# scjjb/HIPT_ABMIL_ATEC23

Measured on AMD Instinct MI355X. Metric: 4K-regions/sec HIPT extract + ABMIL fwd ms @100k×384; 1/2/4/8 MI355X, higher is better.
Workload: dtype bf16; 1 GPU; per step: HIPT_4K.forward on R resident [3,4096,4096] fp32 regions (R x 256 patches ViT-256 -> ViT-4K over each 16x16 [CLS] grid, BASELINE configs[2]) + CLAM_SB gated-attention pooling over one 100000x384 bag (configs[3], the bag resident in the compute dtype); random-init weights of the reference architectures; streams=3, input=fp32 normalised, bag_dtype=bf16-resident, chunk_patches=2048, parallelism=slide-sharded x1, one all-gather

## Files before the change

### hipt_abmil_atec23_amd/_native.py

```python
from __future__ import annotations

import ctypes as C
import os
import subprocess
import threading

HERE = os.path.dirname(os.path.abspath(__file__))
LIB_PATH = os.environ.get("HIPT_AMD_LIB") or os.path.join(HERE, "libhipt_abmil.so")
CSRC = os.path.join(HERE, "csrc")

HIPT_F32, HIPT_BF16 = 0, 1
EPI_GELU, EPI_RESID, EPI_OUT_F32, EPI_RELU = 1, 2, 4, 16
ABI_VERSION = 6
PACK_QKV, PACK_PROJ, PACK_MLP, PACK_QKV_ATT, PACK_CLS_ABSORB = 0, 1, 2, 3, 4
CLS_ABSORB_TAIL = 0x4B564142

c_f32p = C.c_void_p


class BlockWeights(C.Structure):
    _fields_ = [(n, C.c_void_p) for n in (
        "ln1_w", "ln1_b", "qkv_w", "qkv_b", "proj_w", "proj_b",
        "ln2_w", "ln2_b", "fc1_w", "fc1_b", "fc2_w", "fc2_b", "qkv_pk", "proj_pk", "mlp_pk")] + [
        ("mlp_pk_fmt", C.c_int32), ("cls_absorb", C.c_int32), ("qkv_att_pk", C.c_void_p)]
# ... 69 lines not shown
    "hipt_abi_version": (_i, []),
    "hipt_last_error": (C.c_char_p, []),
    "hipt_profile_enable": (_i, [_i]),
    "hipt_profile_categories": (_i, []),
    "hipt_profile_category_name": (C.c_char_p, [_i]),
    "hipt_profile_read": (_i, [_p, _p]),
    "hipt_layernorm": (_i, [_p, _i64, _p, _p, _p, _i, _i64, _i, _i, _f, _p]),
    "hipt_linear": (_i, [_p, _i64, _p, _i64, _p, _p, _p, _i64, _i, _i, _i, _i, _i, _p]),
    "hipt_attention": (_i, [_p, _p, _p, _i, _i, _i, _i, _f, _i, _p]),
    "hipt_vit_workspace_bytes": (_sz, [_VW, _i]),
    "hipt_vit_packed_bytes": (_sz, [_VW, _i]),
    "hipt_vit_mlp_pack_format": (_i, [_VW]),
    "hipt_vit_pack_weights": (_i, [_VW, _i, _i, _p, _p]),
    "hipt_vit256_forward_workspace_bytes": (_sz, [_VW, _IL, _i, _i]),
    "hipt_vit4k_forward_workspace_bytes": (_sz, [_VW, _i]),
    "hipt_vit256_prepare_tokens": (_i, [_VW, _p, _IL, _i, _i, _p, _p, _sz, _p]),
    "hipt_vit4k_prepare_tokens": (_i, [_VW, _p, _i, _p, _p, _sz, _p]),
    "hipt_vit_blocks": (_i, [_VW, _p, _i, _i, _i, _p, _p, _sz, _p]),
    "hipt_vit_head": (_i, [_VW, _p, _i, _i, _p, _p]),
    "hipt_vit_cls_attention": (_i, [_VW, _p, _i, _p, _p, _sz, _p]),
    "hipt_vit_attention_unit": (_i, [_VW, _i, _p, _i, _p, _i, _p, _sz, _p]),
    "hipt_vit_mlp_unit": (_i, [_VW, _i, _p, _p, _i, _p, _p, _sz, _p]),
    "hipt_vit_cls_block_unit": (_i, [_VW, _p, _p, _i, _p, _p, _p, _sz, _p]),
    "hipt_vit_embed_unit": (_i, [_VW, _p, _i, _IL, _i, _i, _p, _p, _p, _sz, _p]),
    "hipt_vit256_forward": (_i, [_VW, _p, _IL, _i, _i, _p, _p, _sz, _p]),
    "hipt_vit4k_forward": (_i, [_VW, _p, _i, _p, _p, _sz, _p]),
    "hipt_image_compute_bytes": (_sz, [_VW, _IL, _i, _i]),
    "hipt_image_to_compute": (_i, [_VW, _p, _i, _IL, _i, _p, _p]),
    "hipt_vit256_range_workspace_bytes": (_sz, [_VW, _i, _i]),
    "hipt_vit256_forward_range": (_i, [_VW, _p, _IL, _i, _i, _i, _p, _p, _sz, _p]),
    "hipt_vit256_range_px_workspace_bytes": (_sz, [_VW, _IL, _i, _i]),
    "hipt_vit256_forward_range_px": (_i, [_VW, _p, _IL, _i, _i, _i, _p, _p, _sz, _p]),
    "hipt_hipt4k_workspace_bytes": (_sz, [_VW, _VW, _i, _i, _i, _i]),
    "hipt_hipt4k_forward": (_i, [_VW, _VW, _p, _i, _i, _i, _i, _p, _p, _p, _sz, _p]),
    "hipt_hipt4k_u8_workspace_bytes": (_sz, [_VW, _VW, _i, _i, _i, _i]),
    "hipt_hipt4k_forward_u8": (_i, [_VW, _VW, _p, _i, _i, _i, _i, _i, _p, _p, _p, _sz, _p]),
    "hipt_u8_normalize": (_i, [_p, _i, C.c_int64, C.c_int64, _p, _i, _p]),
    "hipt_clam_workspace_bytes": (_sz, [_CW, _i]),
    "hipt_clam_stream_packed_bytes": (_sz, [_CW]),
    "hipt_clam_stream_pack": (_i, [_CW, _p, _p]),
    "hipt_clam_ticket_offset": (_sz, [_CW, _i]),
    "hipt_clam_sb_forward": (_i, [_CW, _p, _i, _i, _p, _p, _p, _p, _p, _p, _sz, _p]),
    "hipt_clam_bags_supported": (_i, [_CW]),
    "hipt_clam_bags_workspace_bytes": (_sz, [_CW, _i, _i64]),
    "hipt_clam_sb_forward_bags": (_i, [_CW, _p, _p, _i, _i64, _i, _p, _p, _p, _p, _p, _p, _sz, _p]),
    "hipt_clam_wide_bags_supported": (_i, [_CW]),
# ... 183 lines not shown
```

### hipt_abmil_atec23_amd/csrc/capi.hip

```cpp
#include <stdarg.h>
#include <stdio.h>
#include <stdlib.h>
#include <string.h>

#include "common.h"
#include "kernels.h"
#include "workspace.h"

static thread_local char g_err[512] = "";

void hipt_set_error(const char* fmt, ...) {
    va_list ap;
    va_start(ap, fmt);
    vsnprintf(g_err, sizeof(g_err), fmt, ap);
    va_end(ap);
}

namespace {

inline int esz(int dtype) { return dtype == HIPT_F32 ? 4 : 2; }
inline hipStream_t S(void* s) { return (hipStream_t)s; }

enum { PC_EMBED, PC_LN, PC_QKV, PC_ATTN, PC_PROJ, PC_FC1, PC_FC2, PC_MLP, PC_ABMIL, PC_COMBINE, PC_OTHER, PC_VIT4K, PC_LASTCLS, PC_QKVATT, PC_CLSROWS, PC_N };
const char* const kProfNames[PC_N] = {"embed_gemm", "layernorm", "qkv_gemm", "attention", "proj_gemm",
// ... 90 lines not shown
    const hipt_block_weights& b = w->blocks[blk];
    const int D = w->dim;
    SeqGemmParams q;
    memset(&q, 0, sizeof(q));
    q.M = M; q.K = D; q.ln_eps = w->ln_eps;
    q.A = x; q.lda = D; q.ln_w = b.ln1_w; q.ln_b = b.ln1_b; q.W = b.qkv_w; q.wpk = b.qkv_pk; q.N = 3 * D; q.bias = b.qkv_b;
    q.out = s.qkv; q.ldc = 3 * D; q.out_ntok = w->ntok;
    q.counter = s.queues->qkv;
    return q;
}
inline void qkv_from_xn(SeqGemmParams& q, const void* xn) { q.A = xn, q.ln_w = q.ln_b = nullptr; }

MlpParams mlp_params(const hipt_vit_weights* w, int blk, int M, float* x, const BlockScratch& s) {
    const hipt_block_weights& b = w->blocks[blk];
    MlpParams m;
    memset(&m, 0, sizeof(m));
    m.x = x; m.y1 = s.xn; m.bproj = b.proj_b; m.ln_w = b.ln2_w; m.ln_b = b.ln2_b; m.ln_eps = w->ln_eps;
    m.w1 = b.fc1_w; m.b1 = b.fc1_b; m.w2 = b.fc2_w; m.b2 = b.fc2_b; m.wpk = b.mlp_pk; m.wpk_fmt = b.mlp_pk_fmt; m.M = M; m.D = w->dim; m.hidden = w->hidden;
    m.counter = s.queues->mlp;
    return m;
}
inline void mlp_emit_xn(MlpParams& m, const hipt_block_weights& next, void* xn_out) { m.ln_next_w = next.ln1_w, m.ln_next_b = next.ln1_b, m.xn_out = xn_out; }

int rows_linear(GemmParams p, int dtype, int flags, hipStream_t st, int a_row_step = 0, void* gather = nullptr) {
    p.asc = 1;
    if (a_row_step > 0) {
        if (!hipt_generic_only() && hipt_gemm_arows_supported(p.M, p.K, dtype, ALOAD_PLAIN, 0)) {
            p.a_row_step = a_row_step;
        } else {
            int rc = hipt_gather_cls_bf16_launch(p.A, gather, p.M, a_row_step, p.K, st, 1);
            if (rc) return rc;
            p.A = gather;
        }
    }
    return linear(p, dtype, flags, st);
}

static bool small_call(const hipt_vit_weights* w, int nseq) { return (int64_t)nseq * w->ntok <= 1088; }

static bool blocks_chain(const hipt_vit_weights* w, int nseq, int b0, int b1) {
    const int D = w->dim, dt = w->dtype;
    bool chain = hipt_seqgemm_supported(dt, D) && hipt_mlp_supported(dt, D, w->hidden) && !small_call(w, nseq) && !hipt_generic_only() &&
                 hipt_mlp16_supported(dt, D, w->hidden) && hipt_seqgemm_pipe_supported(dt, D, 3 * D, false, 0);
    for (int i = b0; i < b1 && chain; ++i) chain = w->blocks[i].qkv_pk && w->blocks[i].proj_pk && w->blocks[i].mlp_pk && (w->blocks[i].mlp_pk_fmt == 2 || w->blocks[i].mlp_pk_fmt == 3);
    return chain;
}

static bool can_prune_last(const hipt_vit_weights* w) {
    return w->dtype == HIPT_BF16 && w->dim == 384 && w->dim / w->heads == 64 && w->ntok <= 320 && hipt_seqgemm_supported(w->dtype, w->dim) &&
           hipt_mlp_supported(w->dtype, w->dim, w->hidden) && !hipt_env_on("HIPT_NO_PRUNE");
}

enum {
    RT_EMIT_LAST = 1,
    RT_CLS_ONLY = 2,
    RT_PX_EMBED = 4,
    RT_FORCE_SMALL = 8,
};
struct VitRoute {
    int b0, b1;
    bool emit_last;
    bool small, force_small;
    bool seq;
    bool chain;
    bool img;
    bool hm;
    bool prune;
    bool pre;
    bool fuse_ok, fold_ok, absorb_ok;
    bool have_xn = false;
    bool x_img = false;
};

VitRoute vit_route(const hipt_vit_weights* w, int nseq, int b0, int b1, bool want_probs, int accept) {
    const int D = w->dim, dt = w->dtype;
    const int64_t M = (int64_t)nseq * w->ntok;
    VitRoute r;
    r.force_small = (accept & RT_FORCE_SMALL) != 0;
    r.small = small_call(w, nseq) || r.force_small;
    r.prune = (accept & RT_CLS_ONLY) && can_prune_last(w) && !small_call(w, nseq);
    r.b0 = b0;
    r.b1 = r.prune ? w->depth - 1 : b1;
    r.emit_last = r.prune || (accept & RT_EMIT_LAST);
    r.seq = hipt_seqgemm_supported(dt, D) && hipt_mlp_supported(dt, D, w->hidden) && !r.small;
    r.chain = !r.force_small && blocks_chain(w, nseq, r.b0, r.b1);
    r.img = r.chain && r.prune && !want_probs && M % 16 == 0 && !hipt_env_on("HIPT_NO_IMG") && hipt_attention64_supported(dt, D / w->heads, w->ntok, false);
    r.hm = r.img && M * 3 * D * 2 < ((int64_t)1 << 32) - 65536;
    r.pre = r.img && (accept & RT_PX_EMBED) && r.b0 < r.b1 && !hipt_env_on("HIPT_NO_EMBED_LN");
    r.fuse_ok = hipt_qkv_attn_supported(dt, D, w->heads, w->ntok) && !hipt_env_on("HIPT_NO_FUSED_ATTN");
    r.fold_ok = r.chain && !hipt_env_on("HIPT_NO_PROJ_FOLD");
    r.absorb_ok = hipt_cls_pool_supported(dt, D, w->heads, w->ntok) && !hipt_env_on("HIPT_NO_CLS_ABSORB");
    return r;
}

struct BlockRoute {
    bool fuse;
    bool fold;
    bool absorb;
};
BlockRoute block_route(const VitRoute& r, const hipt_block_weights& b, bool last_probs) {
    BlockRoute k;
    k.fuse = r.have_xn && r.x_img && b.qkv_att_pk && r.fuse_ok && !last_probs;
    k.fold = r.fold_ok && b.mlp_pk_fmt == 3 && !last_probs;
    k.absorb = k.fuse && b.cls_absorb == HIPT_CLS_ABSORB_TAIL && r.absorb_ok;
    return k;
}

int cls_rows_qkv(const hipt_vit_weights* w, const hipt_block_weights& b, int nseq, int N, const BlockScratch& s, int a_row_step, hipStream_t st) {
    const int D = w->dim;
    return rows_linear(gemm_params(a_row_step > 0 ? s.att : s.cls_xn, D, b.qkv_w, D, b.qkv_b, s.cls_qkv, N, nseq, N, D), w->dtype, 0, st, a_row_step, s.cls_xn);
}

int run_blocks(const hipt_vit_weights* w, float* x, int nseq, float* probs, const BlockScratch& s, VitRoute& r, hipStream_t st) {
    const int D = w->dim, M = nseq * w->ntok, dt = w->dtype, dh = D / w->heads;
// ... 44 lines not shown
        }
        const bool ln_al = (((uintptr_t)b.ln1_w | (uintptr_t)b.ln1_b | (uintptr_t)b.ln2_w | (uintptr_t)b.ln2_b) & 15) == 0;
        const bool ln_in_gemm = r.small && ln_al && !hipt_generic_only() && hipt_gemm_ln_supported(M, D, ALOAD_PLAIN, 0, r.force_small);
        auto lin = [&](int cat, GemmParams g, int flags) -> int {
            g.rpt = w->ntok;
            g.small_any = r.force_small ? 1 : 0;
            if (flags & HIPT_EPI_RESID) g.resid = x;
            PROF(cat, linear(g, dt, flags, st));
            return HIPT_OK;
        };
        auto ln_lin = [&](int cat, const float* lw, const float* lb, GemmParams g, int flags) -> int {
            if (ln_in_gemm) {
                g.ln_w = lw; g.ln_b = lb; g.ln_eps = w->ln_eps;
            } else {
                PROF(PC_LN, hipt_layernorm_launch(x, D, lw, lb, s.xn, dt, D, M, D, w->ln_eps, st));
                g.A = s.xn;
            }
            return lin(cat, g, flags);
        };
        const int H = w->hidden;
        if ((rc = ln_lin(PC_QKV, b.ln1_w, b.ln1_b, gemm_params(x, D, b.qkv_w, D, b.qkv_b, s.qkv, 3 * D, M, 3 * D, D), 0))) return rc;
        PROF(PC_ATTN, hipt_attention_launch(s.qkv, s.att, last_probs ? probs : nullptr, nseq, w->ntok, w->heads, dh, scale, dt, st));
        if (last_probs) break;
        if ((rc = lin(PC_PROJ, gemm_params(s.att, D, b.proj_w, D, b.proj_b, x, D, M, D, D), HIPT_EPI_RESID | HIPT_EPI_OUT_F32))) return rc;
        if ((rc = ln_lin(PC_FC1, b.ln2_w, b.ln2_b, gemm_params(x, D, b.fc1_w, D, b.fc1_b, s.hid, H, M, H, D), HIPT_EPI_GELU))) return rc;
        if ((rc = lin(PC_FC2, gemm_params(s.hid, H, b.fc2_w, H, b.fc2_b, x, D, M, D, H), HIPT_EPI_RESID | HIPT_EPI_OUT_F32))) return rc;
    }
    return HIPT_OK;
}

static int run_last_block_cls(const hipt_vit_weights* w, float* x, int nseq, const BlockScratch& s, const VitRoute& r, hipStream_t st) {
    const int D = w->dim, M = nseq * w->ntok, dt = w->dtype, last = w->depth - 1;
    const hipt_block_weights& b = w->blocks[last];
    const float scale = attn_scale(w);
    const BlockRoute k = block_route(r, b, false);
    int rc;
    const void* att_rows = s.att;
    if (k.fuse) {
        PROF(PC_LASTCLS, hipt_gather_cls_bf16_launch(s.att, s.cls_xn, nseq, w->ntok, D, st, 1));
        if (k.absorb) {
            const int HD = w->heads * D;
            const char* wu = (const char*)b.qkv_att_pk + hipt_qkv_attn_packed_bytes();
            const char* wo = wu + (size_t)HD * D * 2;
            PROF(PC_LASTCLS, cls_rows_qkv(w, b, nseq, D, s, 0, st));
            PROF(PC_LASTCLS, rows_linear(gemm_params(s.cls_qkv, D, wu, D, nullptr, s.u, HD, nseq, HD, D), dt, HIPT_EPI_OUT_F32, st));
            PROF(PC_LASTCLS, hipt_cls_pool_launch(s.att, (const float*)s.u, s.z, nseq, scale, st));
            PROF(PC_LASTCLS, rows_linear(gemm_params(s.z, HD, wo, HD, b.qkv_b + 2 * D, s.qkv, D, nseq, D, HD), dt, 0, st));
        } else {
            PROF(PC_LASTCLS, cls_rows_qkv(w, b, nseq, 3 * D, s, 0, st));
            PROF(PC_LASTCLS, hipt_qkv_attn_cls_launch(s.att, b.qkv_att_pk, b.qkv_b, s.cls_qkv, s.qkv, nseq, scale, st));
        }
        att_rows = s.qkv;
    } else {
        SeqGemmParams q = qkv_params(w, last, M, x, s);
        if (r.have_xn) {
            PROF(PC_LASTCLS, hipt_gather_cls_bf16_launch(s.att, s.cls_xn, nseq, w->ntok, D, st, r.x_img ? 1 : 0));
            const size_t wq = (size_t)D * D * 2;
            qkv_from_xn(q, s.att);
            q.img = r.x_img ? 1 : 0;
            q.W = (const char*)b.qkv_w + wq; q.wpk = b.qkv_pk ? (const char*)b.qkv_pk + wq : nullptr; q.N = 2 * D; q.bias = b.qkv_b + D;
            q.out = (bf16_t*)s.qkv + D;
            PROF(PC_LASTCLS, hipt_seqgemm_launch(q, false, 0, st));
            q.img = 0;
            q.M = nseq; q.A = s.cls_xn; q.W = b.qkv_w; q.wpk = b.qkv_pk; q.N = D; q.bias = b.qkv_b; q.out = s.qkv; q.ldc = w->ntok * 3 * D;
            q.counter = s.queues->aux;
            PROF(PC_LASTCLS, hipt_seqgemm_launch(q, false, 0, st));
        } else {
            PROF(PC_QKV, hipt_seqgemm_launch(q, true, 0, st));
        }
        PROF(PC_LASTCLS, hipt_attn_cls_launch(s.qkv, s.att, nullptr, nseq, w->ntok, w->heads, D / w->heads, scale, st));
    }
    PROF(PC_OTHER, hipt_gather_cls_launch(x, s.xc, nseq, (int64_t)w->ntok * D, D, st, r.x_img ? 1 : 0));
    PROF(PC_LASTCLS, rows_linear(gemm_params(att_rows, D, b.proj_w, D, b.proj_b, s.xn, D, nseq, D, D), dt, 0, st));
    PROF(PC_LASTCLS, hipt_mlp_launch(mlp_params(w, last, nseq, s.xc, s), st));
    return HIPT_OK;
}

int64_t image_elems(const hipt_image_layout* lay, int nseq_total) {
    const int per = lay->grid_w * lay->grid_h;
    return (int64_t)((nseq_total + per - 1) / per) * lay->batch_stride;
}

enum { IMG_F32 = 0, IMG_U8_CHW = 1, IMG_U8_HWC = 2 };

size_t image_compute_bytes(const hipt_vit_weights* w, const hipt_image_layout* lay, int nseq, int kind) {
    const size_t n = (size_t)image_elems(lay, nseq);
    return w->dtype == HIPT_BF16 ? al256(n * 2) : kind != IMG_F32 ? al256(n * 4) : 0;
}

int embed256(const hipt_vit_weights* w, const void* img, const hipt_image_layout* lay, int seq0, int nseq, float* x,
             hipStream_t st) {
    HIPT_CHECK_ARG(lay->patch_h % 16 == 0 && lay->patch_w % 16 == 0, "vit256: patch %dx%d not a multiple of 16", lay->patch_h,
                   lay->patch_w);
    const int nty = lay->patch_h / 16, ntx = lay->patch_w / 16;
// ... 308 lines not shown
    m.y1 = att_img;
    m.fold = 1;
    m.img = 3;
    if (xn_out_img) mlp_emit_xn(m, w->blocks[block + 1 < w->depth ? block + 1 : block], xn_out_img);
    hipStream_t st = S(stream);
    PROF(PC_MLP, hipt_mlp_launch(m, st));
    return HIPT_OK;
}

int hipt_vit_cls_block_unit(const hipt_vit_weights* w, const void* xn_img, const float* x_img, int nseq, float* xc_out, void* att_out, void* workspace,
                            size_t ws_bytes, void* stream) {
    int rc = check_vit(w);
    if (rc) return rc;
    HIPT_CHECK_ARG(xn_img && x_img && xc_out && nseq > 0, "vit_cls_block_unit: null/empty argument");
    const int D = w->dim;
    const int64_t M = (int64_t)nseq * w->ntok;
    VitRoute r = vit_route(w, nseq, 0, w->depth, false, RT_CLS_ONLY | RT_PX_EMBED);
    if (!hipt_qkv_attn_supported(w->dtype, D, w->heads, w->ntok) || M % 16 != 0 || !r.prune || !r.chain || !r.img) {
        hipt_set_error("vit_cls_block_unit: bf16, D = 384, 6 heads, 257 tokens, nseq * 257 %% 16 == 0 and a forward that prunes its last block "
                       "on activation images only");
        return HIPT_E_UNSUPPORTED;
    }
    r.have_xn = r.x_img = true;
    Carver c(workspace, workspace ? ws_bytes : 0);
    BlockScratch s = carve_vit4k(c, w, nseq, false).s;
    if ((rc = check_workspace(c, "vit_cls_block_unit"))) return rc;
    HIPT_CHECK_ARG(s.fits_cls_xn, "vit_cls_block_unit: hidden %d leaves no room for the [CLS] rows in the block scratch", w->hidden);
    hipStream_t st = S(stream);
    if (block_route(r, w->blocks[w->depth - 1], false).fuse)
        s.att = const_cast<void*>(xn_img);
    else if (hipMemcpyAsync(s.att, xn_img, (size_t)M * D * 2, hipMemcpyDeviceToDevice, st) != hipSuccess)
        return HIPT_E_LAUNCH;
    const void* rows = s.att == xn_img ? s.qkv : s.att;
    if ((rc = run_last_block_cls(w, const_cast<float*>(x_img), nseq, s, r, st))) return rc;
    if (hipMemcpyAsync(xc_out, s.xc, (size_t)nseq * D * 4, hipMemcpyDeviceToDevice, st) != hipSuccess) return HIPT_E_LAUNCH;
    if (att_out && hipMemcpyAsync(att_out, rows, (size_t)nseq * D * 2, hipMemcpyDeviceToDevice, st) != hipSuccess) return HIPT_E_LAUNCH;
    return HIPT_OK;
}

int hipt_vit_embed_unit(const hipt_vit_weights* w, const void* images, int input_kind, const hipt_image_layout* lay, int seq0, int nseq, float* x_out,
                        void* xn_out_img, void* workspace, size_t ws_bytes, void* stream) {
    int rc = check_vit(w);
    if (rc) return rc;
    HIPT_CHECK_ARG(images && lay && x_out && nseq > 0 && seq0 >= 0 && input_kind >= IMG_F32 && input_kind <= IMG_U8_HWC && (!xn_out_img || w->depth > 0),
                   "vit_embed_unit: bad argument");
    if (!embed_fused_ok(w, images, lay, embed_px_slot_bytes(), input_kind) || (xn_out_img && ((int64_t)nseq * w->ntok) % 16 != 0)) {
        hipt_set_error("vit_embed_unit: bf16, D = 384, 256 x 256 patches of 16 x 16-pixel tokens, 16-byte aligned pixel rows (uint8: strides %% 8 == 0, "
                       "batch_stride = 3 * chan_stride), nseq * ntok %% 16 == 0 for the image outputs, and not under HIPT_GENERIC only");
        return HIPT_E_UNSUPPORTED;
    }
    Carver c(workspace, workspace ? ws_bytes : 0);
    void* slot = c.take(embed_px_slot_bytes());
    if ((rc = check_workspace(c, "vit_embed_unit"))) return rc;
    hipStream_t st = S(stream);
    if ((rc = hipt_embed32_pack_launch(w->embed_w, slot, st))) return rc;
    return embed256_px(w, images, input_kind, lay, seq0, nseq, x_out, slot, xn_out_img, st);
}

int hipt_vit_mlp_pack_format(const hipt_vit_weights* w) { return w && hipt_mlp16_supported(w->dtype, w->dim, w->hidden) ? 3 : 0; }
// ... 47 lines not shown
}

static int vit256_range_impl(const hipt_vit_weights* w, const void* img, const hipt_image_layout* lay, int seq0, int nseq, int chunk, float* out,
                             void* workspace, size_t ws_bytes, hipStream_t st, const void* embed_pk = nullptr, int embed_kind = IMG_F32) {
    int rc;
    const int D = w->dim;
    Carver c(workspace, ws_bytes);
    const RangeWs g = carve_range(c, w, nseq, chunk);
    if ((rc = check_workspace(c, "vit256_forward"))) return rc;
    for (int s0 = 0; s0 < nseq; s0 += g.chunk) {
        const int n = nseq - s0 < g.chunk ? nseq - s0 : g.chunk;
        VitRoute r = vit_route(w, n, 0, w->depth, false, RT_CLS_ONLY | (embed_pk ? RT_PX_EMBED : 0));
        if (r.prune && !(r.chain ? g.s.fits_cls_xn : g.s.fits_xc)) {
            hipt_set_error("vit256_forward: %d tokens x hidden %d leave no room in the block scratch for the [CLS] rows of the pruned last block "
                           "(HIPT_NO_PRUNE=1 runs it in full)", w->ntok, w->hidden);
            return HIPT_E_WORKSPACE;
        }
        if (embed_pk)
            rc = embed256_px(w, img, embed_kind, lay, seq0 + s0, n, g.x, embed_pk, r.pre ? g.s.att : nullptr, st);
        else
            rc = embed256(w, img, lay, seq0 + s0, n, g.x, st);
        if (rc) return rc;
        if ((rc = run_blocks(w, g.x, n, nullptr, g.s, r, st))) return rc;
        if (r.prune && (rc = run_last_block_cls(w, g.x, n, g.s, r, st))) return rc;
        PROF(PC_LN, hipt_layernorm_launch(r.prune ? g.s.xc : g.x, r.prune ? D : (int64_t)w->ntok * D, w->norm_w, w->norm_b, out + (size_t)s0 * D,
                                          HIPT_F32, D, n, D, w->ln_eps, st));
    }
    return HIPT_OK;
}

static int image_to_compute(const hipt_vit_weights* w, const void* images, int kind, const hipt_image_layout* lay, int nseq, void* dst,
                            const void** img_out, hipStream_t st) {
    int rc;
    const int64_t n_img = image_elems(lay, nseq);
    if (kind != IMG_F32) {
        const int per = lay->grid_w * lay->grid_h;
        HIPT_CHECK_ARG(nseq % per == 0, "vit256_forward: uint8 input must hold whole regions");
        const int64_t plane = lay->batch_stride / 3;
        PROF(PC_OTHER, hipt_u8_normalize_launch(images, kind == IMG_U8_HWC, nseq / per, plane, dst, w->dtype, st));
        *img_out = dst;
    } else if (w->dtype == HIPT_BF16) {
        PROF(PC_OTHER, hipt_f32_to_bf16_launch((const float*)images, dst, n_img, st));
        *img_out = dst;
    } else {
        *img_out = images;
    }
    return HIPT_OK;
// ... 363 lines not shown
```

### hipt_abmil_atec23_amd/csrc/kernels.h

```cpp
#pragma once
#include <hip/hip_runtime.h>
#include <stdint.h>

#include "../../include/hipt_abmil.h"

enum { ALOAD_PLAIN = 0, ALOAD_IM2COL = 1 };
enum { EPI_ROWMAP = 32 };

struct GemmParams {
    const void* A;
    int64_t lda;
    const void* W;
    int64_t ldw;
    int M, N, K;
    int rpt;
    const float* bias;
    const float* resid;
    void* out;
    int64_t ldc;
    const float* pos;
    int rows_per_seq;
    hipt_image_layout im;
    int im_nty, im_ntx, im_seq0;
    const float *ln_w, *ln_b;
// ... 88 lines not shown
bool hipt_mlp16_supported(int dtype, int D, int hidden);
int hipt_mlp16_launch(const MlpParams& p, hipStream_t st);
size_t hipt_mlp16_packed_bytes(int D, int hidden, bool with_proj);
int hipt_mlp16_pack_launch(const void* w1, const void* w2, int D, int hidden, void* packed, hipStream_t st, const void* wproj = nullptr);

int hipt_layernorm_launch(const float* x, int64_t x_stride, const float* w, const float* b, void* out, int out_dtype,
                          int64_t out_stride, int rows, int D, float eps, hipStream_t st);

int hipt_attention_launch(const void* qkv, void* out, float* probs, int B, int ntok, int heads, int dh, float scale,
                          int dtype, hipStream_t st, int out_img = 0, int qkv_hm = 0);
bool hipt_attention64_supported(int dtype, int dh, int ntok, bool want_probs);
int hipt_attention64_launch(const void* qkv, void* out, int B, int ntok, int heads, float scale, hipStream_t st, int out_img = 0, int qkv_hm = 0);

bool hipt_qkv_attn_supported(int dtype, int D, int heads, int ntok);
size_t hipt_qkv_attn_packed_bytes();
int hipt_qkv_attn_pack_launch(const void* qkv_w, void* packed, hipStream_t st);
int hipt_qkv_attn_launch(const void* xn_img, const void* wpk, const float* qkv_b, const void* qkv_cls, void* out_img, int nseq, float scale, hipStream_t st);
int hipt_qkv_attn_cls_launch(const void* xn_img, const void* wpk, const float* qkv_b, const void* qkv_cls, void* out_rows, int nseq, float scale, hipStream_t st);

bool hipt_cls_pool_supported(int dtype, int D, int heads, int ntok);
size_t hipt_cls_absorb_packed_bytes();
int hipt_cls_absorb_pack_launch(const void* qkv_w, void* packed, hipStream_t st);
int hipt_cls_pool_launch(const void* xn_img, const float* u, void* z, int nseq, float scale, hipStream_t st);

int hipt_attn_cls_launch(const void* qkv, void* out, float* probs, int B, int ntok, int heads, int dh, float scale, hipStream_t st);
int hipt_attn_cls_probs_launch(const void* qkv, float* probs, int B, int ntok, int heads, int dh, float scale, int dtype, hipStream_t st);
int hipt_gather_cls_launch(const float* src, float* dst, int nseq, int64_t seq_stride, int D, hipStream_t st, int img = 0);
int hipt_gather_cls_bf16_launch(const void* src, void* dst, int nseq, int ntok, int D, hipStream_t st, int img = 0);
int hipt_cls_init_launch(float* x, const float* cls, const float* pos, int nseq, int ntok, int D, hipStream_t st);
int hipt_cls_init_img_launch(float* x_img, void* xn_img, const float* cls, const float* pos, const float* ln_w, const float* ln_b, float ln_eps, int nseq,
                             int ntok, int D, hipStream_t st);
int hipt_add_bf16_launch(float* out, const float* src, const void* y, int64_t n, hipStream_t st);
int hipt_u8_normalize_launch(const void* src, int hwc, int64_t nimg, int64_t plane, void* dst, int dst_dtype, hipStream_t st);
int hipt_f32_to_bf16_launch(const float* in, void* out, int64_t n, hipStream_t st);

bool hipt_clam_fused_supported(const hipt_clam_weights* w);
int hipt_clam_fused_launch(const hipt_clam_weights* w, const void* bag, int N, int attention_only, float* A_raw,
                           float* partials, int* n_partials, hipStream_t st);
bool hipt_clam_stream_supported(const hipt_clam_weights* w);
size_t hipt_clam_stream_image_bytes(const hipt_clam_weights* w);
int hipt_clam_stream_pack_launch(const hipt_clam_weights* w, void* out, hipStream_t st);
int hipt_clam_stream_launch(const hipt_clam_weights* w, const void* bag, int N, int attention_only, float* A_raw,
                            float* partials, int* n_partials, unsigned* ticket, float* M, float* logits, float* Y_prob,
                            int64_t* Y_hat, hipStream_t st);
bool hipt_clam_mb_stream_supported(const hipt_clam_weights* w);
size_t hipt_clam_mb_h1_bytes(int N);
// ... 36 lines not shown
```

### include/hipt_abmil.h

```cpp
#ifndef HIPT_ABMIL_H
#define HIPT_ABMIL_H

#include <stddef.h>
#include <stdint.h>

#ifdef __cplusplus
extern "C" {
#endif

#define HIPT_ABI_VERSION 6

enum { HIPT_F32 = 0, HIPT_BF16 = 1 };

enum {
    HIPT_OK = 0,
    HIPT_E_BADARG = -1,
    HIPT_E_WORKSPACE = -2,
    HIPT_E_LAUNCH = -3,
    HIPT_E_UNSUPPORTED = -4
};

int hipt_abi_version(void);
const char* hipt_last_error(void);

// ... 69 lines not shown
size_t hipt_vit256_forward_workspace_bytes(const hipt_vit_weights* w, const hipt_image_layout* lay,
                                           int nseq, int chunk);
size_t hipt_vit4k_forward_workspace_bytes(const hipt_vit_weights* w, int nseq);

int hipt_vit256_prepare_tokens(const hipt_vit_weights* w, const float* images,
                               const hipt_image_layout* lay, int seq0, int nseq, float* x,
                               void* workspace, size_t ws_bytes, void* stream);

int hipt_vit4k_prepare_tokens(const hipt_vit_weights* w, const float* tokens_in, int nseq, float* x,
                              void* workspace, size_t ws_bytes, void* stream);

int hipt_vit_blocks(const hipt_vit_weights* w, float* x, int nseq, int blk_begin, int blk_end,
                    float* probs, void* workspace, size_t ws_bytes, void* stream);

int hipt_vit_attention_unit(const hipt_vit_weights* w, int block, const void* xn_img, int nseq, void* out_img, int fused,
                            void* workspace, size_t ws_bytes, void* stream);

int hipt_vit_mlp_unit(const hipt_vit_weights* w, int block, float* x_img, const void* att_img, int nseq, void* xn_out_img,
                      void* workspace, size_t ws_bytes, void* stream);

int hipt_vit_cls_block_unit(const hipt_vit_weights* w, const void* xn_img, const float* x_img, int nseq, float* xc_out, void* att_out,
                            void* workspace, size_t ws_bytes, void* stream);

int hipt_vit_embed_unit(const hipt_vit_weights* w, const void* images, int input_kind, const hipt_image_layout* lay, int seq0, int nseq,
                        float* x_out, void* xn_out_img, void* workspace, size_t ws_bytes, void* stream);

int hipt_vit_cls_attention(const hipt_vit_weights* w, float* x, int nseq, float* probs_cls,
                           void* workspace, size_t ws_bytes, void* stream);

int hipt_vit_head(const hipt_vit_weights* w, const float* x, int nseq, int cls_only, float* out,
                  void* stream);

int hipt_vit256_forward(const hipt_vit_weights* w, const float* images, const hipt_image_layout* lay,
                        int nseq, int chunk, float* out, void* workspace, size_t ws_bytes, void* stream);

size_t hipt_image_compute_bytes(const hipt_vit_weights* w, const hipt_image_layout* lay, int nseq, int input_kind);
int hipt_image_to_compute(const hipt_vit_weights* w, const void* images, int input_kind, const hipt_image_layout* lay,
                          int nseq, void* dst, void* stream);
size_t hipt_vit256_range_workspace_bytes(const hipt_vit_weights* w, int nseq, int chunk);
int hipt_vit256_forward_range(const hipt_vit_weights* w, const void* images_cd, const hipt_image_layout* lay,
                              int seq0, int nseq, int chunk, float* out, void* workspace, size_t ws_bytes, void* stream);
size_t hipt_vit256_range_px_workspace_bytes(const hipt_vit_weights* w, const hipt_image_layout* lay, int nseq, int chunk);
int hipt_vit256_forward_range_px(const hipt_vit_weights* w, const float* images, const hipt_image_layout* lay, int seq0, int nseq,
                                 int chunk, float* out, void* workspace, size_t ws_bytes, void* stream);

int hipt_vit4k_forward(const hipt_vit_weights* w, const float* tokens_in, int nseq, float* out,
// ... 306 lines not shown
```

Before: 339.5 regions/s.

## Fuse proj, LN2, MLP and final norm into one per-row chain kernel

Adds a row_chain kernel that runs, for 16-row tiles, the attention output projection with residual, LayerNorm2, FC1+GELU, FC2 with residual, and optionally a leading absorbed-value GEMM and the final norm, keeping intermediates in LDS. It is used for the small ViT-4K block path and the last-block CLS rows of ViT-256, replacing several GEMM, gather and layernorm launches. The aim is to cut launch overhead and intermediate memory traffic on the small-M stages. The cost is that each block streams the full weight matrices for only 16 rows, so weight reuse is low and few workgroups are launched for small M.

```diff
diff --git a/hipt_abmil_atec23_amd/_native.py b/hipt_abmil_atec23_amd/_native.py
--- a/hipt_abmil_atec23_amd/_native.py
+++ b/hipt_abmil_atec23_amd/_native.py
@@ -115,6 +115,7 @@
     "hipt_vit_attention_unit": (_i, [_VW, _i, _p, _i, _p, _i, _p, _sz, _p]),
     "hipt_vit_mlp_unit": (_i, [_VW, _i, _p, _p, _i, _p, _p, _sz, _p]),
     "hipt_vit_cls_block_unit": (_i, [_VW, _p, _p, _i, _p, _p, _p, _sz, _p]),
+    "hipt_row_chain_unit": (_i, [_VW, _i, _p, _p, _p, _p, _i64, _i, _i, _p, _i, _p]),
     "hipt_vit_embed_unit": (_i, [_VW, _p, _i, _IL, _i, _i, _p, _p, _p, _sz, _p]),
     "hipt_vit256_forward": (_i, [_VW, _p, _IL, _i, _i, _p, _p, _sz, _p]),
     "hipt_vit4k_forward": (_i, [_VW, _p, _i, _p, _p, _sz, _p]),
diff --git a/hipt_abmil_atec23_amd/csrc/capi.hip b/hipt_abmil_atec23_amd/csrc/capi.hip
--- a/hipt_abmil_atec23_amd/csrc/capi.hip
+++ b/hipt_abmil_atec23_amd/csrc/capi.hip
@@ -136,6 +136,15 @@
 }
 inline void mlp_emit_xn(MlpParams& m, const hipt_block_weights& next, void* xn_out) { m.ln_next_w = next.ln1_w, m.ln_next_b = next.ln1_b, m.xn_out = xn_out; }
 
+RowChainParams chain_params(const hipt_vit_weights* w, const hipt_block_weights& b, int M, const void* a, const float* x, int64_t x_row_step, int x_img, float* out) {
+    RowChainParams c;
+    memset(&c, 0, sizeof(c));
+    c.a = a; c.lda = w->dim; c.x = x; c.x_row_step = x_row_step; c.x_img = x_img; c.out = out; c.M = M;
+    c.proj_w = b.proj_w; c.proj_b = b.proj_b; c.ln_w = b.ln2_w; c.ln_b = b.ln2_b; c.ln_eps = w->ln_eps;
+    c.fc1_w = b.fc1_w; c.fc1_b = b.fc1_b; c.fc2_w = b.fc2_w; c.fc2_b = b.fc2_b;
+    return c;
+}
+
 int rows_linear(GemmParams p, int dtype, int flags, hipStream_t st, int a_row_step = 0, void* gather = nullptr) {
     p.asc = 1;
     if (a_row_step > 0) {
@@ -182,6 +191,7 @@
     bool prune;
     bool pre;
     bool fuse_ok, fold_ok, absorb_ok;
+    bool row_chain;
     bool have_xn = false;
     bool x_img = false;
 };
@@ -204,6 +214,7 @@
     r.fuse_ok = hipt_qkv_attn_supported(dt, D, w->heads, w->ntok) && !hipt_env_on("HIPT_NO_FUSED_ATTN");
     r.fold_ok = r.chain && !hipt_env_on("HIPT_NO_PROJ_FOLD");
     r.absorb_ok = hipt_cls_pool_supported(dt, D, w->heads, w->ntok) && !hipt_env_on("HIPT_NO_CLS_ABSORB");
+    r.row_chain = hipt_row_chain_supported(dt, D, w->hidden) && !hipt_generic_only() && !hipt_env_on("HIPT_NO_ROW_CHAIN");
     return r;
 }
 
@@ -294,6 +305,13 @@
         if ((rc = ln_lin(PC_QKV, b.ln1_w, b.ln1_b, gemm_params(x, D, b.qkv_w, D, b.qkv_b, s.qkv, 3 * D, M, 3 * D, D), 0))) return rc;
         PROF(PC_ATTN, hipt_attention_launch(s.qkv, s.att, last_probs ? probs : nullptr, nseq, w->ntok, w->heads, dh, scale, dt, st));
         if (last_probs) break;
+        if (r.force_small && r.row_chain) {
+            const RowChainParams c = chain_params(w, b, M, s.att, x, 1, 0, x);
+            if (hipt_row_chain_aligned(c)) {
+                PROF(PC_VIT4K, hipt_row_chain_launch(c, D, st));
+                continue;
+            }
+        }
         if ((rc = lin(PC_PROJ, gemm_params(s.att, D, b.proj_w, D, b.proj_b, x, D, M, D, D), HIPT_EPI_RESID | HIPT_EPI_OUT_F32))) return rc;
         if ((rc = ln_lin(PC_FC1, b.ln2_w, b.ln2_b, gemm_params(x, D, b.fc1_w, D, b.fc1_b, s.hid, H, M, H, D), HIPT_EPI_GELU))) return rc;
         if ((rc = lin(PC_FC2, gemm_params(s.hid, H, b.fc2_w, H, b.fc2_b, x, D, M, D, H), HIPT_EPI_RESID | HIPT_EPI_OUT_F32))) return rc;
@@ -301,13 +319,17 @@
     return HIPT_OK;
 }
 
-static int run_last_block_cls(const hipt_vit_weights* w, float* x, int nseq, const BlockScratch& s, const VitRoute& r, hipStream_t st) {
+static int run_last_block_cls(const hipt_vit_weights* w, float* x, int nseq, const BlockScratch& s, const VitRoute& r, hipStream_t st,
+                              float* norm_out = nullptr, bool* normed = nullptr) {
     const int D = w->dim, M = nseq * w->ntok, dt = w->dtype, last = w->depth - 1;
     const hipt_block_weights& b = w->blocks[last];
     const float scale = attn_scale(w);
     const BlockRoute k = block_route(r, b, false);
     int rc;
     const void* att_rows = s.att;
+    RowChainParams c = chain_params(w, b, nseq, nullptr, x, w->ntok, r.x_img ? 1 : 0, norm_out ? norm_out : s.xc);
+    if (norm_out) c.norm_w = w->norm_w, c.norm_b = w->norm_b;
+    bool chain = r.row_chain;
     if (k.fuse) {
         PROF(PC_LASTCLS, hipt_gather_cls_bf16_launch(s.att, s.cls_xn, nseq, w->ntok, D, st, 1));
         if (k.absorb) {
@@ -317,6 +339,12 @@
             PROF(PC_LASTCLS, cls_rows_qkv(w, b, nseq, D, s, 0, st));
             PROF(PC_LASTCLS, rows_linear(gemm_params(s.cls_qkv, D, wu, D, nullptr, s.u, HD, nseq, HD, D), dt, HIPT_EPI_OUT_F32, st));
             PROF(PC_LASTCLS, hipt_cls_pool_launch(s.att, (const float*)s.u, s.z, nseq, scale, st));
+            c.a = s.z; c.lda = HD; c.lead_w = wo; c.lead_ldw = HD; c.lead_b = b.qkv_b + 2 * D; c.dh = D / w->heads;
+            if ((chain = chain && hipt_row_chain_aligned(c))) {
+                PROF(PC_LASTCLS, hipt_row_chain_launch(c, D, st));
+                if (normed) *normed = norm_out != nullptr;
+                return HIPT_OK;
+            }
             PROF(PC_LASTCLS, rows_linear(gemm_params(s.z, HD, wo, HD, b.qkv_b + 2 * D, s.qkv, D, nseq, D, HD), dt, 0, st));
         } else {
             PROF(PC_LASTCLS, cls_rows_qkv(w, b, nseq, 3 * D, s, 0, st));
@@ -342,6 +370,12 @@
         }
         PROF(PC_LASTCLS, hipt_attn_cls_launch(s.qkv, s.att, nullptr, nseq, w->ntok, w->heads, D / w->heads, scale, st));
     }
+    c.a = att_rows; c.lda = D; c.lead_w = nullptr; c.lead_b = nullptr;
+    if (chain && hipt_row_chain_aligned(c)) {
+        PROF(PC_LASTCLS, hipt_row_chain_launch(c, D, st));
+        if (normed) *normed = norm_out != nullptr;
+        return HIPT_OK;
+    }
     PROF(PC_OTHER, hipt_gather_cls_launch(x, s.xc, nseq, (int64_t)w->ntok * D, D, st, r.x_img ? 1 : 0));
     PROF(PC_LASTCLS, rows_linear(gemm_params(att_rows, D, b.proj_w, D, b.proj_b, s.xn, D, nseq, D, D), dt, 0, st));
     PROF(PC_LASTCLS, hipt_mlp_launch(mlp_params(w, last, nseq, s.xc, s), st));
@@ -696,6 +730,7 @@
         return HIPT_E_UNSUPPORTED;
     }
     r.have_xn = r.x_img = true;
+    r.row_chain = false;
     Carver c(workspace, workspace ? ws_bytes : 0);
     BlockScratch s = carve_vit4k(c, w, nseq, false).s;
     if ((rc = check_workspace(c, "vit_cls_block_unit"))) return rc;
@@ -709,6 +744,24 @@
     if ((rc = run_last_block_cls(w, const_cast<float*>(x_img), nseq, s, r, st))) return rc;
     if (hipMemcpyAsync(xc_out, s.xc, (size_t)nseq * D * 4, hipMemcpyDeviceToDevice, st) != hipSuccess) return HIPT_E_LAUNCH;
     if (att_out && hipMemcpyAsync(att_out, rows, (size_t)nseq * D * 2, hipMemcpyDeviceToDevice, st) != hipSuccess) return HIPT_E_LAUNCH;
+    return HIPT_OK;
+}
+
+int hipt_row_chain_unit(const hipt_vit_weights* w, int block, const void* a, const void* lead_w, const float* lead_b, const float* x, int64_t x_row_step,
+                        int x_img, int final_norm, float* out, int M, void* stream) {
+    int rc = check_vit(w);
+    if (rc) return rc;
+    HIPT_CHECK_ARG(block >= 0 && block < w->depth && a && x && out && M > 0, "row_chain_unit: bad argument");
+    if (!hipt_row_chain_supported(w->dtype, w->dim, w->hidden)) {
+        hipt_set_error("row_chain_unit: bf16, D in {192, 384}, hidden = 4 D only (dtype %d, D = %d, hidden = %d)", w->dtype, w->dim, w->hidden);
+        return HIPT_E_UNSUPPORTED;
+    }
+    const int D = w->dim;
+    RowChainParams c = chain_params(w, w->blocks[block], M, a, x, x_row_step, x_img, out);
+    if (lead_w) c.lda = c.lead_ldw = (int64_t)w->heads * D, c.lead_w = lead_w, c.lead_b = lead_b, c.dh = D / w->heads;
+    if (final_norm) c.norm_w = w->norm_w, c.norm_b = w->norm_b;
+    hipStream_t st = S(stream);
+    PROF(D >= 384 ? PC_LASTCLS : PC_VIT4K, hipt_row_chain_launch(c, D, st));
     return HIPT_OK;
 }
 
@@ -802,7 +855,9 @@
             rc = embed256(w, img, lay, seq0 + s0, n, g.x, st);
         if (rc) return rc;
         if ((rc = run_blocks(w, g.x, n, nullptr, g.s, r, st))) return rc;
-        if (r.prune && (rc = run_last_block_cls(w, g.x, n, g.s, r, st))) return rc;
+        bool normed = false;
+        if (r.prune && (rc = run_last_block_cls(w, g.x, n, g.s, r, st, out + (size_t)s0 * D, &normed))) return rc;
+        if (normed) continue;
         PROF(PC_LN, hipt_layernorm_launch(r.prune ? g.s.xc : g.x, r.prune ? D : (int64_t)w->ntok * D, w->norm_w, w->norm_b, out + (size_t)s0 * D,
                                           HIPT_F32, D, n, D, w->ln_eps, st));
     }
diff --git a/hipt_abmil_atec23_amd/csrc/kernels.h b/hipt_abmil_atec23_amd/csrc/kernels.h
--- a/hipt_abmil_atec23_amd/csrc/kernels.h
+++ b/hipt_abmil_atec23_amd/csrc/kernels.h
@@ -134,6 +134,32 @@
 size_t hipt_cls_absorb_packed_bytes();
 int hipt_cls_absorb_pack_launch(const void* qkv_w, void* packed, hipStream_t st);
 int hipt_cls_pool_launch(const void* xn_img, const float* u, void* z, int nseq, float scale, hipStream_t st);
+
+struct RowChainParams {
+    const void*   a;
+    int64_t lda;
+    const void*   lead_w;
+    int64_t lead_ldw;
+    const float* lead_b;
+    int dh;
+    const float* x;
+    int64_t x_row_step;
+    int x_img;
+    const void*   proj_w;
+    const float* proj_b;
+    const float *ln_w, *ln_b;
+    float ln_eps;
+    const void*   fc1_w;
+    const float* fc1_b;
+    const void*   fc2_w;
+    const float* fc2_b;
+    const float *norm_w, *norm_b;
+    float* out;
+    int M;
+};
+bool hipt_row_chain_supported(int dtype, int D, int hidden);
+bool hipt_row_chain_aligned(const RowChainParams& p);
+int hipt_row_chain_launch(const RowChainParams& p, int D, hipStream_t st);
 
 int hipt_attn_cls_launch(const void* qkv, void* out, float* probs, int B, int ntok, int heads, int dh, float scale, hipStream_t st);
 int hipt_attn_cls_probs_launch(const void* qkv, float* probs, int B, int ntok, int heads, int dh, float scale, int dtype, hipStream_t st);
diff --git a/hipt_abmil_atec23_amd/csrc/row_chain.hip b/hipt_abmil_atec23_amd/csrc/row_chain.hip
--- /dev/null
+++ b/hipt_abmil_atec23_amd/csrc/row_chain.hip
@@ -0,0 +1,262 @@
+#include "common.h"
+#include "kernels.h"
+#include "launch.h"
+#include "mlp_common.h"
+
+namespace {
+
+constexpr int RC_NT = 3;
+
+template <int D> struct RcCfg {
+    static constexpr int H = 4 * D, WAVES = D / (16 * RC_NT), THREADS = 64 * WAVES;
+    static constexpr int APITCH = D * 2 + 16, HPITCH = H * 2 + 16;
+    static constexpr int OFF_H = 16 * APITCH, OFF_ST = OFF_H + 16 * HPITCH, LDS = OFF_ST + 2 * WAVES * 16 * 4;
+    static_assert(D % (16 * RC_NT) == 0 && LDS <= 64 * 1024, "static LDS");
+};
+
+template <int NK, bool AG>
+__device__ __forceinline__ void rc_mm(f32x4 (&acc)[RC_NT], const bf16_t* const (&wp)[RC_NT], const char* const (&ap)[RC_NT]) {
+    constexpr int KU = (NK % 12 == 0 && !AG) ? 6 : 3;
+    static_assert(NK % (2 * KU) == 0, "two register sets in turn");
+    constexpr int NA = AG ? RC_NT : 1;
+    u32x4 w0[KU][RC_NT], w1[KU][RC_NT], a0[KU][NA], a1[KU][NA];
+    auto load = [&](u32x4(&w)[KU][RC_NT], u32x4(&a)[KU][NA], int k0) {
+#pragma unroll
+        for (int d = 0; d < KU; ++d) {
+#pragma unroll
+            for (int t = 0; t < RC_NT; ++t) w[d][t] = *(const u32x4*)(wp[t] + (k0 + d) * 32);
+            if constexpr (AG) {
+#pragma unroll
+                for (int t = 0; t < RC_NT; ++t) a[d][t] = *(const u32x4*)(ap[t] + (k0 + d) * 64);
+            }
+        }
+    };
+    auto mma = [&](const u32x4(&w)[KU][RC_NT], const u32x4(&a)[KU][NA], int k0) {
+#pragma unroll
+        for (int d = 0; d < KU; ++d) {
+            if constexpr (AG) {
+#pragma unroll
+                for (int t = 0; t < RC_NT; ++t) Tr<bf16_t>::mma16(acc[t], w[d][t], a[d][t]);
+            } else {
+                const u32x4 al = *(const u32x4*)(ap[0] + (k0 + d) * 64);
+#pragma unroll
+                for (int t = 0; t < RC_NT; ++t) Tr<bf16_t>::mma16(acc[t], w[d][t], al);
+            }
+        }
+    };
+    load(w0, a0, 0);
+    for (int k0 = 0; k0 < NK; k0 += 2 * KU) {
+        load(w1, a1, k0 + KU);
+        mma(w0, a0, k0);
+        if (k0 + 2 * KU < NK) load(w0, a0, k0 + 2 * KU);
+        mma(w1, a1, k0 + KU);
+    }
+}
+
+template <int D, bool ERF>
+__global__ __launch_bounds__(RcCfg<D>::THREADS) void row_chain_kernel(const RowChainParams p) {
+    using C = RcCfg<D>;
+    constexpr int H = C::H, WAVES = C::WAVES;
+    __shared__ __attribute__((aligned(16))) char smem[C::LDS];
+    const int tid = threadIdx.x, lane = tid & 63, li = lane & 15, g = lane >> 4;
+    const int w = __builtin_amdgcn_readfirstlane(tid >> 6);
+    const int row0 = blockIdx.x * 16;
+    const int row = row0 + li < p.M ? row0 + li : p.M - 1;
+    char* const abuf = smem;
+    char* const hbuf = smem + C::OFF_H;
+    float* const st = (float*)(smem + C::OFF_ST);
+    const int nw = 16 * RC_NT * w;
+
+    f32x4 xr[RC_NT];
+    {
+        const int64_t R = (int64_t)row * p.x_row_step;
+#pragma unroll
+        for (int t = 0; t < RC_NT; ++t) {
+            const int n = nw + 16 * t + 4 * g;
+            if (p.x_img) {
+                const int m = n >> 3;
+                xr[t] = *(const f32x4*)(p.x + (R >> 4) * (16 * D) + (m >> 2) * 512 + ((n >> 2) & 1) * 256 + (16 * (m & 3) + (int)(R & 15)) * 4);
+            } else {
+                xr[t] = *(const f32x4*)(p.x + R * D + n);
+            }
+        }
+    }
+
+    if (p.lead_w) {
+        f32x4 acc[RC_NT];
+        const bf16_t* wp[RC_NT];
+        const char* ap[RC_NT];
+#pragma unroll
+        for (int t = 0; t < RC_NT; ++t) {
+            const int n0 = nw + 16 * t, k0 = (n0 / p.dh) * D;
+            acc[t] = f32x4{0.f, 0.f, 0.f, 0.f};
+            wp[t] = (const bf16_t*)p.lead_w + (int64_t)(n0 + li) * p.lead_ldw + k0 + 8 * g;
+            ap[t] = (const char*)((const bf16_t*)p.a + (int64_t)row * p.lda + k0 + 8 * g);
+        }
+        rc_mm<D / 32, true>(acc, wp, ap);
+#pragma unroll
+        for (int t = 0; t < RC_NT; ++t) {
+            const int n = nw + 16 * t + 4 * g;
+            const f32x4 v = acc[t] + *(const f32x4*)(p.lead_b + n);
+            u32x2 o;
+            o[0] = pack_bf16x2(v[0], v[1]), o[1] = pack_bf16x2(v[2], v[3]);
+            *(u32x2*)(abuf + li * C::APITCH + n * 2) = o;
+        }
+    } else {
+        for (int i = tid; i < 16 * (D / 8); i += C::THREADS) {
+            const int r = i / (D / 8), c = i % (D / 8);
+            const int rr = row0 + r < p.M ? row0 + r : p.M - 1;
+            *(u32x4*)(abuf + r * C::APITCH + c * 16) = *(const u32x4*)((const bf16_t*)p.a + (int64_t)rr * p.lda + c * 8);
+        }
+    }
+    __syncthreads();
+
+    const char* const arow[RC_NT] = {abuf + li * C::APITCH + 16 * g, nullptr, nullptr};
+    const char* const hrow[RC_NT] = {hbuf + li * C::HPITCH + 16 * g, nullptr, nullptr};
+
+    {
+        f32x4 acc[RC_NT];
+        const bf16_t* wp[RC_NT];
+#pragma unroll
+        for (int t = 0; t < RC_NT; ++t) {
+            acc[t] = f32x4{0.f, 0.f, 0.f, 0.f};
+            wp[t] = (const bf16_t*)p.proj_w + (int64_t)(nw + 16 * t + li) * D + 8 * g;
+        }
+        rc_mm<D / 32, false>(acc, wp, arow);
+#pragma unroll
+        for (int t = 0; t < RC_NT; ++t) xr[t] += acc[t] + *(const f32x4*)(p.proj_b + nw + 16 * t + 4 * g);
+    }
+
+    auto row_stats = [&](float& mean, float& rstd) {
+        float s = 0.f;
+#pragma unroll
+        for (int t = 0; t < RC_NT; ++t) s += (xr[t][0] + xr[t][1]) + (xr[t][2] + xr[t][3]);
+        s += __shfl_xor(s, 16, 64);
+        s += __shfl_xor(s, 32, 64);
+        if (g == 0) st[w * 16 + li] = s;
+        __syncthreads();
+        float tot = 0.f;
+#pragma unroll
+        for (int v = 0; v < WAVES; ++v) tot += st[v * 16 + li];
+        mean = tot / (float)D;
+        float q = 0.f;
+#pragma unroll
+        for (int t = 0; t < RC_NT; ++t)
+#pragma unroll
+            for (int e = 0; e < 4; ++e) {
+                const float c = xr[t][e] - mean;
+                q += c * c;
+            }
+        q += __shfl_xor(q, 16, 64);
+        q += __shfl_xor(q, 32, 64);
+        if (g == 0) st[(WAVES + w) * 16 + li] = q;
+        __syncthreads();
+        float qt = 0.f;
+#pragma unroll
+        for (int v = 0; v < WAVES; ++v) qt += st[(WAVES + v) * 16 + li];
+        rstd = 1.0f / sqrtf(qt / (float)D + p.ln_eps);
+    };
+
+    {
+        float mean, rstd;
+        row_stats(mean, rstd);
+#pragma unroll
+        for (int t = 0; t < RC_NT; ++t) {
+            const int n = nw + 16 * t + 4 * g;
+            const f32x4 gm = *(const f32x4*)(p.ln_w + n), bt = *(const f32x4*)(p.ln_b + n);
+            f32x4 o;
+#pragma unroll
+            for (int e = 0; e < 4; ++e) o[e] = (xr[t][e] - mean) * rstd * gm[e] + bt[e];
+            u32x2 ob;
+            ob[0] = pack_bf16x2(o[0], o[1]), ob[1] = pack_bf16x2(o[2], o[3]);
+            *(u32x2*)(abuf + li * C::APITCH + n * 2) = ob;
+        }
+    }
+    __syncthreads();
+
+    for (int q = 0; q < H / (16 * RC_NT * WAVES); ++q) {
+        const int nh = 16 * RC_NT * (q * WAVES + w);
+        f32x4 acc[RC_NT];
+        const bf16_t* wp[RC_NT];
+#pragma unroll
+        for (int t = 0; t < RC_NT; ++t) {
+            acc[t] = f32x4{0.f, 0.f, 0.f, 0.f};
+            wp[t] = (const bf16_t*)p.fc1_w + (int64_t)(nh + 16 * t + li) * D + 8 * g;
+        }
+        rc_mm<D / 32, false>(acc, wp, arow);
+#pragma unroll
+        for (int t = 0; t < RC_NT; ++t) {
+            const int n = nh + 16 * t + 4 * g;
+            f32x4 v = acc[t] + *(const f32x4*)(p.fc1_b + n);
+#pragma unroll
+            for (int e = 0; e < 4; ++e) v[e] = ERF ? gelu_erf(v[e]) : gelu1(v[e]);
+            u32x2 o;
+            o[0] = pack_bf16x2(v[0], v[1]), o[1] = pack_bf16x2(v[2], v[3]);
+            *(u32x2*)(hbuf + li * C::HPITCH + n * 2) = o;
+        }
+    }
+    __syncthreads();
+
+    {
+        f32x4 acc[RC_NT];
+        const bf16_t* wp[RC_NT];
+#pragma unroll
+        for (int t = 0; t < RC_NT; ++t) {
+            acc[t] = f32x4{0.f, 0.f, 0.f, 0.f};
+            wp[t] = (const bf16_t*)p.fc2_w + (int64_t)(nw + 16 * t + li) * H + 8 * g;
+        }
+        rc_mm<H / 32, false>(acc, wp, hrow);
+#pragma unroll
+        for (int t = 0; t < RC_NT; ++t) xr[t] += acc[t] + *(const f32x4*)(p.fc2_b + nw + 16 * t + 4 * g);
+    }
+
+    if (p.norm_w) {
+        float mean, rstd;
+        row_stats(mean, rstd);
+#pragma unroll
+        for (int t = 0; t < RC_NT; ++t) {
+            const int n = nw + 16 * t + 4 * g;
+            const f32x4 gm = *(const f32x4*)(p.norm_w + n), bt = *(const f32x4*)(p.norm_b + n);
+#pragma unroll
+            for (int e = 0; e < 4; ++e) xr[t][e] = (xr[t][e] - mean) * rstd * gm[e] + bt[e];
+        }
+    }
+    if (row0 + li < p.M) {
+#pragma unroll
+        for (int t = 0; t < RC_NT; ++t) *(f32x4*)(p.out + (int64_t)(row0 + li) * D + nw + 16 * t + 4 * g) = xr[t];
+    }
+}
+
+inline bool al16(const void* q) { return ((uintptr_t)q & 15) == 0; }
+
+}
+
+bool hipt_row_chain_supported(int dtype, int D, int hidden) { return dtype == HIPT_BF16 && (D == 192 || D == 384) && hidden == 4 * D; }
+
+bool hipt_row_chain_aligned(const RowChainParams& p) {
+    return al16(p.a) && al16(p.x) && al16(p.out) && al16(p.proj_w) && al16(p.proj_b) && al16(p.ln_w) && al16(p.ln_b) && al16(p.fc1_w) && al16(p.fc1_b) &&
+           al16(p.fc2_w) && al16(p.fc2_b) && al16(p.lead_w) && al16(p.lead_b) && al16(p.norm_w) && al16(p.norm_b) && p.lda % 8 == 0 && p.lead_ldw % 8 == 0;
+}
+
+int hipt_row_chain_launch(const RowChainParams& p, int D, hipStream_t st) {
+    HIPT_CHECK_ARG(D == 192 || D == 384, "row_chain: D = %d (192 and 384 only)", D);
+    HIPT_CHECK_ARG(p.M > 0 && p.a && p.x && p.out && p.proj_w && p.proj_b && p.ln_w && p.ln_b && p.fc1_w && p.fc1_b && p.fc2_w && p.fc2_b, "row_chain: null/empty argument");
+    HIPT_CHECK_ARG(hipt_row_chain_aligned(p), "row_chain: operands off the 16-byte grid");
+    HIPT_CHECK_ARG((p.norm_w != nullptr) == (p.norm_b != nullptr), "row_chain: the final norm needs weight and bias");
+    HIPT_CHECK_ARG(p.x_row_step >= 1 && (!p.x_img || D == 384), "row_chain: residual rows: step %lld, image %d (images are 384 wide)", (long long)p.x_row_step, p.x_img);
+    if (p.lead_w)
+        HIPT_CHECK_ARG(p.lead_b && p.dh > 0 && p.dh % 16 == 0 && D % p.dh == 0 && p.lead_ldw >= (int64_t)(D / p.dh) * D && p.lda >= (int64_t)(D / p.dh) * D,
+                       "row_chain: leading GEMM: head width %d, row pitches %lld / %lld", p.dh, (long long)p.lead_ldw, (long long)p.lda);
+    else
+        HIPT_CHECK_ARG(p.lda >= D, "row_chain: attention rows of pitch %lld", (long long)p.lda);
+    HIPT_CHECK_ARG((const void*)p.out != (const void*)p.x || (p.x_row_step == 1 && !p.x_img), "row_chain: in place needs row-major rows of step 1");
+    static DeviceSetup setup;
+    if (int rc = setup({}, 0, "row_chain")) return rc;
+    const dim3 grid((p.M + 15) / 16);
+    if (D == 192)
+        hipLaunchKernelGGL((row_chain_kernel<192, true>), grid, dim3(RcCfg<192>::THREADS), 0, st, p);
+    else
+        hipLaunchKernelGGL((row_chain_kernel<384, false>), grid, dim3(RcCfg<384>::THREADS), 0, st, p);
+    HIPT_CHECK_LAUNCH();
+    return HIPT_OK;
+}
diff --git a/include/hipt_abmil.h b/include/hipt_abmil.h
--- a/include/hipt_abmil.h
+++ b/include/hipt_abmil.h
@@ -115,6 +115,9 @@
 int hipt_vit_cls_block_unit(const hipt_vit_weights* w, const void* xn_img, const float* x_img, int nseq, float* xc_out, void* att_out,
                             void* workspace, size_t ws_bytes, void* stream);
 
+int hipt_row_chain_unit(const hipt_vit_weights* w, int block, const void* a, const void* lead_w, const float* lead_b, const float* x,
+                        int64_t x_row_step, int x_img, int final_norm, float* out, int M, void* stream);
+
 int hipt_vit_embed_unit(const hipt_vit_weights* w, const void* images, int input_kind, const hipt_image_layout* lay, int seq0, int nseq,
                         float* x_out, void* xn_out_img, void* workspace, size_t ws_bytes, void* stream);
 
```

Result: no change. 340.2 regions/s (median of 6 runs) (+0.2%).
